# YannDubs/lossyless

Hardware: AMD Instinct MI355X
Metric: encode_img_per_sec (higher is better)
Workload: dtype f16; 1 GPU; clip_compressor_b005 encode, synthetic 224x224x3 fp16 NHWC, batch=1024/GPU (configs[1]); batch_per_gpu=1024, layout=nhwc, vit_weights=synthetic-seed1, parallelism=image-parallel x1, entropy_group=16, tower_batch=8704, tower_streams=1, distinct_batches=9

## Files before the change

lossyless_amd/csrc/gemm_w8_kernel.h:

```cpp
#pragma once
#include "gemm_common.h"

namespace lla {
namespace {

constexpr int kWStage = 65536, kWARegion = 32768;
constexpr int kWBiasOff = 2 * kWStage, kWBiasBytes = 3072 * 4;
#ifndef LLA_W8_GROUP_M
#define LLA_W8_GROUP_M 4
#endif
#ifndef LLA_W8_DMA_N0
#define LLA_W8_DMA_N0 5
#endif
#ifndef LLA_W8_DMA_N1
#define LLA_W8_DMA_N1 13
#endif

struct WItem { int kind, idx, d; };
constexpr WItem w_item(int p, int k) {
  return p == 0 ? WItem{0, 2 + k, 1} : p == 1 ? WItem{1, k, 2} : p == 2 ? WItem{1, 2 + k, 2} : WItem{0, k, 2};
}
constexpr int w_confirm(int p) {
  int seq = 0, last_a[14][4] = {}, last_b[14] = {}, upto[14][4] = {};
  for (int t = -2; t < 10; ++t)
    for (int q = 0; q < 4; ++q) {
      for (int k = 0; k < 2; ++k) {
        const WItem it = w_item(q, k);
        const int u = t + it.d;
        ++seq;
        if (u >= 0 && u < 14) { if (it.kind == 0) last_a[u][it.idx] = seq; else last_b[u] = seq; }
      }
      if (t >= 0) upto[t][q] = seq;
    }
  const int t = 4;
  int need = 0;
  if (p == 0) need = last_a[t][2];
  if (p == 1) need = last_a[t][3];
  if (p == 2) need = last_a[t + 1][0] > last_b[t + 1] ? last_a[t + 1][0] : last_b[t + 1];
  if (p == 3) need = last_a[t + 1][1];
  return upto[t][p] - need;
}
static_assert(w_confirm(0) == 9 && w_confirm(1) == 10 && w_confirm(2) == 7 && w_confirm(3) == 8, "schedule / wait counts out of step");
constexpr int w_confirm_pipe(int kind, int p, int n0, int n1) {
  const int TL = 6;
  int seq = 0, last_a[16][4] = {}, last_b[16] = {}, upto[16][4] = {};
  for (int t = 0; t < 12; ++t)
    for (int q = 0; q < 4; ++q) {
      const bool stores = (t == TL && q >= 1) || (t == TL + 1 && q == 0);
      for (int n = 0; n < 16; ++n) {
        if (n == n0 || n == n1) {
          const WItem it = w_item(q, n == n1 ? 1 : 0);
          const int u = t + it.d;
          ++seq;
          if (it.kind == 0) last_a[u][it.idx] = seq; else last_b[u] = seq;
        }
        if (stores && (n & 3) == 3) ++seq;
      }
      upto[t][q] = seq;
    }
  const int t = kind == 1 ? TL : kind == 2 ? TL + 1 : 3;
  int need = 0;
  if (p == 0) need = last_a[t][2];
  if (p == 1) need = last_a[t][3];
  if (p == 2) need = last_a[t + 1][0] > last_b[t + 1] ? last_a[t + 1][0] : last_b[t + 1];
  if (p == 3) need = last_a[t + 1][1];
  return upto[t][p] - need;
}
static_assert(w_confirm_pipe(0, 0, 5, 13) == 9 && w_confirm_pipe(0, 1, 5, 13) == 10 && w_confirm_pipe(0, 2, 5, 13) == 7 &&
              w_confirm_pipe(0, 3, 5, 13) == 8, "the replayed stream and the schedule table must agree where there are no stores");
static_assert(w_confirm_pipe(1, 0, 5, 13) == 9 && w_confirm_pipe(1, 1, 5, 13) == 14 && w_confirm_pipe(1, 2, 5, 13) == 15 &&
              w_confirm_pipe(1, 3, 5, 13) == 20 && w_confirm_pipe(2, 0, 5, 13) == 25 && w_confirm_pipe(2, 1, 5, 13) == 26 &&
              w_confirm_pipe(2, 2, 5, 13) == 14 && w_confirm_pipe(2, 3, 5, 13) == 13, "hand count of the default placement");

template <int... I, class F>
__device__ __forceinline__ void w_static_for_impl(std::integer_sequence<int, I...>, F &&f) { (f(std::integral_constant<int, I>{}), ...); }
template <int N, class F>
__device__ __forceinline__ void w_static_for(F &&f) { w_static_for_impl(std::make_integer_sequence<int, N>{}, f); }

typedef unsigned w_rsrc_t __attribute__((ext_vector_type(4)));
template <int IMM>
__device__ __forceinline__ void w_dma(unsigned voff, w_rsrc_t rsrc, unsigned soff, unsigned lds_base) {
  asm volatile("s_add_u32 m0, %3, %4\n\t"
               "s_nop 0\n\t"
               "buffer_load_dwordx4 %0, %1, %2 offen" LLA_DMA_SC " lds"
               :
               : "v"(voff), "s"(rsrc), "s"(soff), "s"(lds_base), "n"(IMM)
               : "memory", "m0", "scc");
}
__device__ __forceinline__ void w_dma_flat(unsigned voff, const unsigned char *sbase, unsigned lds_dst) {
  asm volatile("s_mov_b32 m0, %2\n\t"
               "s_nop 0\n\t"
               "global_load_lds_dwordx4 %0, %1"
               :
               : "v"(voff), "s"(sbase), "s"(lds_dst)
               : "memory", "m0");
}

#define LLA_W8_WAIT_VM(C) __builtin_amdgcn_s_waitcnt(0x0F70 | ((C) & 15) | (((C) >> 4) << 14))

template <int EPI, int DBG = 0, int PIPE = 0>
__global__ __launch_bounds__(512) void gemm_w8_kernel(GemmParams p) {
  static_assert(EPI == EPI_F16 || EPI == EPI_QGELU, "fp16 outputs only");
  constexpr bool kPipe = PIPE != 0 && DBG == 0;
  kernel_acquire();
  __shared__ __attribute__((aligned(16))) unsigned char smem[kWBiasOff + kWBiasBytes];

  const int tid = threadIdx.x, lane = tid & 63;
  const int wid = __builtin_amdgcn_readfirstlane(tid >> 6);
  const int wr = wid >> 2, wc = wid & 3;
  const int r16 = lane & 15, kq = lane >> 4;

  const int tiles_n = p.N / 256, tiles_m = (p.M + 255) / 256;
  const int total = tiles_m * tiles_n;
  const int bid = blockIdx.x, nblk = gridDim.x;
  const int xcd = bid & 7, slot = bid >> 3;
  const int nslots = (nblk - xcd + 7) >> 3;
  const int tq = total >> 3, tr = total & 7;
  const int start = xcd < tr ? xcd * (tq + 1) : tr * (tq + 1) + (xcd - tr) * tq;
  const int count = tq + (xcd < tr ? 1 : 0);
  const int n_my = slot < count ? (count - slot + nslots - 1) / nslots : 0;
  if (n_my == 0) return;
  constexpr int group_m = LLA_W8_GROUP_M;
  auto tile_origin = [&](int j, int &m0, int &n0) {
    int logical = start + slot + j * nslots;
    if (p.rev) logical = total - 1 - logical;
    const int per_group = group_m * tiles_n;
    const int grp = logical / per_group;
    const int in_grp = logical - grp * per_group;
    const int gh = (tiles_m - grp * group_m) < group_m ? (tiles_m - grp * group_m) : group_m;
    const int tn = in_grp / gh;
    m0 = (grp * group_m + (in_grp - tn * gh)) * 256;
    n0 = tn * 256;
  };
  const int nk = p.K / 64;

  const int pc = lane & 7, lc = pc ^ (((wid & 1) << 2) | (lane >> 4));
  const int rowA = (wid >> 2) * 128 + (wid & 3) * 8 + (lane >> 3);
  const int rowB = wid * 8 + (lane >> 3);
  unsigned voffA[4], voffB[4];
#pragma unroll
  for (int a = 0; a < 4; ++a) {
    voffA[a] = (unsigned)((rowA + 32 * a) * p.lda + lc * 8) * 2u;
    voffB[a] = (unsigned)((rowB + 64 * a) * p.K + lc * 8) * 2u;
  }
  const unsigned lds_base = (unsigned)(uintptr_t)(lptr_t)smem;
  const unsigned dstA = __builtin_amdgcn_readfirstlane(lds_base + (unsigned)((wid >> 2) * 16384 + (wid & 3) * 1024));
  const unsigned dstB = __builtin_amdgcn_readfirstlane(lds_base + (unsigned)(kWARegion + wid * 1024));
  auto make_rsrc = [](const void *base) {
    const unsigned long long a = reinterpret_cast<unsigned long long>(base);
    w_rsrc_t r = {(unsigned)__builtin_amdgcn_readfirstlane((unsigned)a),
                  (unsigned)__builtin_amdgcn_readfirstlane((unsigned)(a >> 32)) & 0xFFFFu, 0xFFFFFFFFu, 0x00020000u};
    return r;
  };
  const w_rsrc_t rsrcA = make_rsrc(p.A), rsrcB = make_rsrc(p.W);
  unsigned srcA[2], srcB[2];
  int cur_j = 0, cur_kt = 0;
  auto src_of = [&](int j, int kt, unsigned &a, unsigned &b) {
    int m0, n0;
    tile_origin(j < n_my ? j : n_my - 1, m0, n0);
    if (m0 + 256 > p.M) m0 = p.M >= 256 ? p.M - 256 : 0;
    a = __builtin_amdgcn_readfirstlane((unsigned)(((size_t)m0 * p.lda + (size_t)kt * 64) * 2));
    b = __builtin_amdgcn_readfirstlane((unsigned)(((size_t)n0 * p.K + (size_t)kt * 64) * 2));
  };
  auto advance_cursor = [&] {
    if (DBG == 15) return;
    srcA[0] = srcA[1]; srcB[0] = srcB[1];
    if (++cur_kt < nk) { srcA[1] += 128; srcB[1] += 128; }
    else { cur_kt = 0; ++cur_j; src_of(cur_j, 0, srcA[1], srcB[1]); }
  };
  if (p.M < 256) {
#pragma unroll
    for (int a = 0; a < 4; ++a) {
      const int r = rowA + 32 * a;
      voffA[a] = (unsigned)((r < p.M ? r : p.M - 1) * p.lda + lc * 8) * 2u;
    }
  }
  auto issue = [&](auto kind_c, auto idx_c, int d, unsigned st_off) {
    constexpr int kind = decltype(kind_c)::value, idx = decltype(idx_c)::value;
    if constexpr (kind == 0) w_dma<idx * 4096>(voffA[idx], rsrcA, srcA[d - 1], dstA + st_off);
    else w_dma<idx * 8192>(voffB[idx], rsrcB, srcB[d - 1], dstB + st_off);
  };
  using I0 = std::integral_constant<int, 0>; using I1 = std::integral_constant<int, 1>;
  using I2 = std::integral_constant<int, 2>; using I3 = std::integral_constant<int, 3>;

  unsigned a_off[2], b_off[2];
#pragma unroll
  for (int s = 0; s < 2; ++s) {
    const unsigned c = (unsigned)(((4 * s + kq) ^ ((r16 >> 1) & 7)) * 16);
    a_off[s] = (unsigned)((wr * 128 + r16) * 128) + c;
    b_off[s] = (unsigned)kWARegion + (unsigned)((wc * 64 + r16) * 128) + c;
  }
  f16x8 gb[4][2], ga[2][2];
  f32x4 acc[8][4];
  auto read_a = [&](unsigned so, int frag, int af, int s) {
    ga[af][s] = *reinterpret_cast<const f16x8 *>(smem + so + a_off[s] + frag * 2048);
  };
  auto read_b = [&](unsigned so, int b, int s) {
    gb[b][s] = *reinterpret_cast<const f16x8 *>(smem + so + b_off[s] + b * 2048);
  };

  if (p.bias) {
    for (int q = wid; q * 256 < p.N; q += 8)
      w_dma_flat((unsigned)lane * 16u, reinterpret_cast<const unsigned char *>(p.bias) + (size_t)q * 1024,
                 __builtin_amdgcn_readfirstlane(lds_base + (unsigned)kWBiasOff + (unsigned)q * 1024u));
  } else {
    for (int i = tid; i * 16 < p.N * 4; i += 512) *reinterpret_cast<f32x4 *>(smem + kWBiasOff + i * 16) = f32x4{0.f, 0.f, 0.f, 0.f};
  }
  src_of(0, 0, srcA[1], srcB[1]);
  srcA[0] = srcA[1]; srcB[0] = srcB[1];
  issue(I0{}, I0{}, 2, 0u); issue(I0{}, I1{}, 2, 0u); issue(I0{}, I2{}, 2, 0u); issue(I0{}, I3{}, 2, 0u);
  issue(I1{}, I0{}, 2, 0u); issue(I1{}, I1{}, 2, 0u); issue(I1{}, I2{}, 2, 0u); issue(I1{}, I3{}, 2, 0u);
  advance_cursor();
  issue(I1{}, I0{}, 2, (unsigned)kWStage); issue(I1{}, I1{}, 2, (unsigned)kWStage);
  issue(I1{}, I2{}, 2, (unsigned)kWStage); issue(I1{}, I3{}, 2, (unsigned)kWStage);
  issue(I0{}, I0{}, 2, (unsigned)kWStage); issue(I0{}, I1{}, 2, (unsigned)kWStage);
  advance_cursor();
  LLA_W8_WAIT_VM(6);
  asm volatile("" ::: "memory");
  __builtin_amdgcn_s_barrier();
  asm volatile("" ::: "memory");
#pragma unroll
  for (int b = 0; b < 4; ++b) read_b(0u, b, 0);
  read_a(0u, 0, 0, 0); read_a(0u, 1, 1, 0); read_a(0u, 0, 0, 1);

  int it = 0;

  typedef unsigned u32x4 __attribute__((ext_vector_type(4)));
  f32x4 ebias[4];
  unsigned char *ecrow = nullptr;
  unsigned elive = 0;
  unsigned ebias_off = 0;
  const size_t e_f_step = (size_t)16 * p.ldc * 2;
  auto epi_setup = [&](int cj) {
    int m0c, n0c;
    tile_origin(cj, m0c, n0c);
    unsigned ones = ~0u;
    asm volatile("" : "+s"(ones));
    const int el = (int)__builtin_amdgcn_mbcnt_hi(ones, __builtin_amdgcn_mbcnt_lo(ones, 0u));
    const int er = el & 15, eq = el >> 4;
    int mbase = m0c, mskip = 0;
    if (m0c + 256 > p.M) { mbase = p.M >= 256 ? p.M - 256 : 0; mskip = m0c - mbase; }
    const int nw = n0c + wc * 64;
    const int rl0 = wr * 128 + er;
    const int col = 16 * (eq & 1) + 8 * (eq >> 1);
    elive = 0;
#pragma unroll
    for (int f = 0; f < 8; ++f) elive |= (rl0 + 16 * f >= mskip && mbase + rl0 + 16 * f < p.M) ? (1u << f) : 0u;
    ecrow = reinterpret_cast<unsigned char *>(reinterpret_cast<f16 *>(p.C) + (size_t)(mbase + rl0) * p.ldc + nw + col);
    ebias_off = (unsigned)(nw + 4 * eq) * 4u;
  };
  auto epi_bias = [&](int b) {
    ebias[b] = *reinterpret_cast<const f32x4 *>(smem + kWBiasOff + ebias_off + 64 * b);
  };
  auto epi_frag = [&](int f) {
    u32x4 o[2];
#pragma unroll
    for (int bp = 0; bp < 4; bp += 2) {
      unsigned lo[2], hi[2];
#pragma unroll
      for (int h = 0; h < 2; ++h) {
        f32x4 v = acc[f][bp + h];
        asm volatile("" : "+v"(v));
        v += ebias[bp + h];
        if constexpr (EPI == EPI_QGELU) {
#pragma unroll
          for (int e = 0; e < 4; ++e) v[e] = quick_gelu(v[e]);
        }
        typedef f16 f16x2 __attribute__((ext_vector_type(2)));
        const f16x2 a2 = {(f16)v[0], (f16)v[1]}, b2 = {(f16)v[2], (f16)v[3]};
        lo[h] = __builtin_bit_cast(unsigned, a2);
        hi[h] = __builtin_bit_cast(unsigned, b2);
      }
      const auto rx = __builtin_amdgcn_permlane16_swap(lo[0], lo[1], false, false);
      const auto ry = __builtin_amdgcn_permlane16_swap(hi[0], hi[1], false, false);
      o[bp >> 1] = u32x4{rx[0], ry[0], rx[1], ry[1]};
    }
    if constexpr (DBG == 5) asm volatile("" ::"v"(o[0]), "v"(o[1]));
    else if ((elive >> f) & 1u) { store16(ecrow + f * e_f_step, o[0]); store16(ecrow + f * e_f_step + 64, o[1]); }
  };

  auto ktile = [&](auto first_c, auto last_c, auto pend_c) {
    constexpr bool FIRST = decltype(first_c)::value, LAST = decltype(last_c)::value, PEND = decltype(pend_c)::value;
    unsigned so = (unsigned)(it & 1) * kWStage, sn = (unsigned)((it + 1) & 1) * kWStage;
    w_static_for<4>([&](auto a_c) {
      constexpr int a = decltype(a_c)::value;
      __builtin_amdgcn_sched_barrier(0);
      if (DBG != 2) __builtin_amdgcn_s_barrier();
      __builtin_amdgcn_sched_barrier(0);
      asm volatile("" : "+s"(so), "+s"(sn));
      w_static_for<16>([&](auto n_c) {
        constexpr int n = decltype(n_c)::value;
        constexpr int g = n >> 2, b = n & 3, s = g >> 1, af = g & 1;
        if constexpr (FIRST && s == 0) {
          const f32x4 zero4 = {0.f, 0.f, 0.f, 0.f};
          acc[2 * a + af][b] = __builtin_amdgcn_mfma_f32_16x16x32_f16(gb[b][0], ga[af][0], zero4, 0, 0, 0);
        } else {
          acc[2 * a + af][b] = __builtin_amdgcn_mfma_f32_16x16x32_f16(gb[b][s], ga[af][s], acc[2 * a + af][b], 0, 0, 0);
        }
        __builtin_amdgcn_sched_barrier(0);
        if constexpr (b == 0) {
          constexpr int pg = (g + 3) & 3, ps = pg >> 1, paf = pg & 1;
          if constexpr (g == 0) read_a(so, 2 * a + paf, paf, ps);
          else if constexpr (a < 3) read_a(so, 2 * (a + 1) + paf, paf, ps);
          else read_a(sn, paf, paf, ps);
        }
        if constexpr (a == 0 && n < 4) read_b(so, n, 1);
        if constexpr (a == 3 && n >= 8 && n < 12) read_b(sn, n - 8, 0);
        if constexpr (DBG != 1 && DBG != 13 && (n == LLA_W8_DMA_N0 || n == LLA_W8_DMA_N1)) {
          constexpr WItem item = w_item(a, n == LLA_W8_DMA_N1 ? 1 : 0);
          issue(std::integral_constant<int, item.kind>{}, std::integral_constant<int, item.idx>{}, item.d,
                (unsigned)((it + item.d) & 1) * kWStage);
        }
        if constexpr (kPipe && (LAST || PEND)) {
          if constexpr (LAST && a == 0) { if constexpr ((n & 3) == 3) epi_bias(n >> 2); }
          else if constexpr ((n & 7) == 7) {
            if constexpr (LAST) epi_frag(2 * (a - 1) + (n >> 3));
            else if constexpr (a == 0) epi_frag(6 + (n >> 3));
          }
        }
        __builtin_amdgcn_sched_barrier(0);
      });
      if (DBG != 4) {
        constexpr int kind = !kPipe ? 0 : LAST ? 1 : PEND ? 2 : 0;
        constexpr int cf = w_confirm_pipe(kind, a, LLA_W8_DMA_N0, LLA_W8_DMA_N1);
        static_assert(cf <= 63, "vmcnt is a 6-bit field");
        LLA_W8_WAIT_VM(cf);
      }
      asm volatile("" ::: "memory");
    });
    ++it;
    advance_cursor();
  };
  using T_ = std::integral_constant<bool, true>;
  using F_ = std::integral_constant<bool, false>;

  for (int cj = 0; cj < n_my; ++cj) {
    if constexpr (kPipe) {
      if (cj == 0) ktile(T_{}, F_{}, F_{});
      else ktile(T_{}, F_{}, T_{});
      for (int kt = 1; kt < nk - 1; ++kt) ktile(F_{}, F_{}, F_{});
      epi_setup(cj);
      ktile(F_{}, T_{}, F_{});
      continue;
    }
    ktile(T_{}, F_{}, F_{});
    for (int kt = 1; kt < nk; ++kt) ktile(F_{}, F_{}, F_{});
    asm volatile("" ::: "memory");
    if constexpr (DBG == 3 || DBG == 13 || DBG == 15) {
      unsigned ones = ~0u;
      asm volatile("" : "+s"(ones));
      const int el = (int)__builtin_amdgcn_mbcnt_hi(ones, __builtin_amdgcn_mbcnt_lo(ones, 0u));
      float t = 0.f;
#pragma unroll
      for (int f = 0; f < 8; ++f)
#pragma unroll
        for (int b = 0; b < 4; ++b) t += acc[f][b][0] + acc[f][b][1] + acc[f][b][2] + acc[f][b][3];
      if (t == 1.2345e30f) reinterpret_cast<f16 *>(p.C)[el] = (f16)t;
    } else {
      epi_setup(cj);
#pragma unroll
      for (int b = 0; b < 4; ++b) epi_bias(b);
#pragma unroll
      for (int f = 0; f < 8; ++f) epi_frag(f);
    }
    asm volatile("" ::: "memory");
  }
  if constexpr (kPipe) {
    epi_frag(6); epi_frag(7);
  }
  __builtin_amdgcn_s_waitcnt(0x0070);
  kernel_release();
}


}
}
```

Baseline: 107,700 img/s.

## Halve workgroup barriers per K-tile in W8 GEMM by re-planning DMA schedule

Cuts the s_barrier and vmcnt waits in the 8-wave GEMM main loop from four per K-tile to two (at phases 1 and 3). The LDS DMA item schedule is reassigned so every write-after-read and read-after-write hazard is still covered by the remaining barriers, and a constexpr replay checks legality and computes the wait counts. The aim is to reduce barrier stalls between waves. In exchange, loads must land earlier and some waits get tighter, and the old four-barrier schedule stays available behind a macro.

```diff
diff --git a/lossyless_amd/csrc/gemm_w8_kernel.h b/lossyless_amd/csrc/gemm_w8_kernel.h
--- a/lossyless_amd/csrc/gemm_w8_kernel.h
+++ b/lossyless_amd/csrc/gemm_w8_kernel.h
@@ -16,61 +16,89 @@
 #define LLA_W8_DMA_N1 13
 #endif
 
+#ifndef LLA_W8_SYNC4
+#define LLA_W8_SYNC4 0
+#endif
+constexpr bool w_meets(int p) { return LLA_W8_SYNC4 ? true : (p & 1) != 0; }
+
 struct WItem { int kind, idx, d; };
+#if LLA_W8_SYNC4
+constexpr int w_nitems(int) { return 2; }
 constexpr WItem w_item(int p, int k) {
   return p == 0 ? WItem{0, 2 + k, 1} : p == 1 ? WItem{1, k, 2} : p == 2 ? WItem{1, 2 + k, 2} : WItem{0, k, 2};
 }
-constexpr int w_confirm(int p) {
-  int seq = 0, last_a[14][4] = {}, last_b[14] = {}, upto[14][4] = {};
-  for (int t = -2; t < 10; ++t)
-    for (int q = 0; q < 4; ++q) {
-      for (int k = 0; k < 2; ++k) {
-        const WItem it = w_item(q, k);
-        const int u = t + it.d;
-        ++seq;
-        if (u >= 0 && u < 14) { if (it.kind == 0) last_a[u][it.idx] = seq; else last_b[u] = seq; }
-      }
-      if (t >= 0) upto[t][q] = seq;
-    }
-  const int t = 4;
-  int need = 0;
-  if (p == 0) need = last_a[t][2];
-  if (p == 1) need = last_a[t][3];
-  if (p == 2) need = last_a[t + 1][0] > last_b[t + 1] ? last_a[t + 1][0] : last_b[t + 1];
-  if (p == 3) need = last_a[t + 1][1];
-  return upto[t][p] - need;
-}
-static_assert(w_confirm(0) == 9 && w_confirm(1) == 10 && w_confirm(2) == 7 && w_confirm(3) == 8, "schedule / wait counts out of step");
-constexpr int w_confirm_pipe(int kind, int p, int n0, int n1) {
+#else
+constexpr int w_nitems(int p) { return p == 0 ? 1 : p == 1 ? 3 : 2; }
+constexpr WItem w_item(int p, int k) {
+  return p == 0 ? WItem{0, 2, 1} : p == 1 ? (k == 0 ? WItem{0, 3, 1} : WItem{1, k - 1, 2}) : p == 2 ? WItem{1, 2 + k, 2} : WItem{0, 1 - k, 2};
+}
+#endif
+constexpr int w_pos(int p, int k, int n0, int n1) {
+  return w_nitems(p) == 1 ? (n0 + n1) / 2 : w_nitems(p) == 2 ? (k == 0 ? n0 : n1) : (k == 0 ? n0 : k == 1 ? (n0 + n1) / 2 : n1);
+}
+constexpr int w_prologue() {
+  int n = 0;
+  for (int p = 0; p < 4; ++p)
+    for (int k = 0; k < w_nitems(p); ++k) n += w_item(p, k).d == 2 ? 1 : 0;
+  return n;
+}
+
+struct WReplay { int cf[4]; bool legal; };
+constexpr WReplay w_replay(int kind, int n0, int n1) {
   const int TL = 6;
-  int seq = 0, last_a[16][4] = {}, last_b[16] = {}, upto[16][4] = {};
+  int seq = 0, stamp[16][8] = {}, upto[64] = {};
+  bool legal = true;
   for (int t = 0; t < 12; ++t)
     for (int q = 0; q < 4; ++q) {
       const bool stores = (t == TL && q >= 1) || (t == TL + 1 && q == 0);
       for (int n = 0; n < 16; ++n) {
-        if (n == n0 || n == n1) {
-          const WItem it = w_item(q, n == n1 ? 1 : 0);
-          const int u = t + it.d;
-          ++seq;
-          if (it.kind == 0) last_a[u][it.idx] = seq; else last_b[u] = seq;
-        }
+        for (int k = 0; k < w_nitems(q); ++k)
+          if (w_pos(q, k, n0, n1) == n) {
+            const WItem it = w_item(q, k);
+            const int u = t + it.d, piece = it.kind == 0 ? it.idx : 4 + it.idx;
+            stamp[u][piece] = ++seq;
+            const int last_read = 4 * (u - 2) + (it.kind == 0 ? it.idx : 0);
+            bool met = false;
+            for (int g = last_read + 1; g <= 4 * t + q; ++g) met = met || w_meets(g & 3);
+            legal = legal && met;
+          }
         if (stores && (n & 3) == 3) ++seq;
       }
-      upto[t][q] = seq;
+      upto[4 * t + q] = seq;
     }
   const int t = kind == 1 ? TL : kind == 2 ? TL + 1 : 3;
-  int need = 0;
-  if (p == 0) need = last_a[t][2];
-  if (p == 1) need = last_a[t][3];
-  if (p == 2) need = last_a[t + 1][0] > last_b[t + 1] ? last_a[t + 1][0] : last_b[t + 1];
-  if (p == 3) need = last_a[t + 1][1];
-  return upto[t][p] - need;
-}
-static_assert(w_confirm_pipe(0, 0, 5, 13) == 9 && w_confirm_pipe(0, 1, 5, 13) == 10 && w_confirm_pipe(0, 2, 5, 13) == 7 &&
-              w_confirm_pipe(0, 3, 5, 13) == 8, "the replayed stream and the schedule table must agree where there are no stores");
-static_assert(w_confirm_pipe(1, 0, 5, 13) == 9 && w_confirm_pipe(1, 1, 5, 13) == 14 && w_confirm_pipe(1, 2, 5, 13) == 15 &&
-              w_confirm_pipe(1, 3, 5, 13) == 20 && w_confirm_pipe(2, 0, 5, 13) == 25 && w_confirm_pipe(2, 1, 5, 13) == 26 &&
-              w_confirm_pipe(2, 2, 5, 13) == 14 && w_confirm_pipe(2, 3, 5, 13) == 13, "hand count of the default placement");
+  WReplay r{{-1, -1, -1, -1}, legal};
+  for (int p = 0; p < 4; ++p) {
+    if (!w_meets((p + 1) & 3)) continue;
+    int need = 0;
+    for (int g = 4 * t + p + 1; g == 4 * t + p + 1 || !w_meets(g & 3); ++g)
+      for (int u = t; u <= t + 2; ++u)
+        for (int piece = 0; piece < 8; ++piece) {
+          const int first_read = 4 * u + (piece < 4 ? piece - 1 : -1);
+          if (first_read != g) continue;
+          if (stamp[u][piece] == 0 || stamp[u][piece] > upto[4 * t + p]) r.legal = false;
+          if (stamp[u][piece] > need) need = stamp[u][piece];
+        }
+    r.cf[p] = upto[4 * t + p] - need;
+    if (need == 0 || r.cf[p] < 0 || r.cf[p] > 63) r.legal = false;
+  }
+  int once[8] = {};
+  for (int q = 0; q < 4; ++q)
+    for (int k = 0; k < w_nitems(q); ++k) ++once[w_item(q, k).kind == 0 ? w_item(q, k).idx : 4 + w_item(q, k).idx];
+  for (int piece = 0; piece < 8; ++piece) r.legal = r.legal && once[piece] == 1;
+  return r;
+}
+constexpr bool w_replay_ok(int n0, int n1) { return w_replay(0, n0, n1).legal && w_replay(1, n0, n1).legal && w_replay(2, n0, n1).legal; }
+static_assert(w_replay_ok(5, 13) && w_replay_ok(2, 10) && w_replay_ok(7, 15), "DMA schedule: a WAR or RAW rule is broken");
+#if LLA_W8_SYNC4
+static_assert(w_replay(0, 5, 13).cf[0] == 9 && w_replay(0, 5, 13).cf[1] == 10 && w_replay(0, 5, 13).cf[2] == 7 &&
+              w_replay(0, 5, 13).cf[3] == 8, "schedule / wait counts out of step");
+static_assert(w_replay(1, 5, 13).cf[0] == 9 && w_replay(1, 5, 13).cf[1] == 14 && w_replay(1, 5, 13).cf[2] == 15 &&
+              w_replay(1, 5, 13).cf[3] == 20 && w_replay(2, 5, 13).cf[0] == 25 && w_replay(2, 5, 13).cf[1] == 26 &&
+              w_replay(2, 5, 13).cf[2] == 14 && w_replay(2, 5, 13).cf[3] == 13, "hand count of the default placement");
+#else
+static_assert(w_replay(0, 5, 13).cf[1] < 0 && w_replay(0, 5, 13).cf[3] < 0, "two periods per K-tile: waits close phases 0 and 2 only");
+#endif
 
 template <int... I, class F>
 __device__ __forceinline__ void w_static_for_impl(std::integer_sequence<int, I...>, F &&f) { (f(std::integral_constant<int, I>{}), ...); }
@@ -211,11 +239,16 @@
   issue(I0{}, I0{}, 2, 0u); issue(I0{}, I1{}, 2, 0u); issue(I0{}, I2{}, 2, 0u); issue(I0{}, I3{}, 2, 0u);
   issue(I1{}, I0{}, 2, 0u); issue(I1{}, I1{}, 2, 0u); issue(I1{}, I2{}, 2, 0u); issue(I1{}, I3{}, 2, 0u);
   advance_cursor();
-  issue(I1{}, I0{}, 2, (unsigned)kWStage); issue(I1{}, I1{}, 2, (unsigned)kWStage);
-  issue(I1{}, I2{}, 2, (unsigned)kWStage); issue(I1{}, I3{}, 2, (unsigned)kWStage);
-  issue(I0{}, I0{}, 2, (unsigned)kWStage); issue(I0{}, I1{}, 2, (unsigned)kWStage);
+  w_static_for<4>([&](auto q_c) {
+    constexpr int q = decltype(q_c)::value;
+    w_static_for<w_nitems(q)>([&](auto k_c) {
+      constexpr WItem item = w_item(q, decltype(k_c)::value);
+      if constexpr (item.d == 2)
+        issue(std::integral_constant<int, item.kind>{}, std::integral_constant<int, item.idx>{}, 2, (unsigned)kWStage);
+    });
+  });
   advance_cursor();
-  LLA_W8_WAIT_VM(6);
+  LLA_W8_WAIT_VM(w_prologue());
   asm volatile("" ::: "memory");
   __builtin_amdgcn_s_barrier();
   asm volatile("" ::: "memory");
@@ -285,7 +318,7 @@
     w_static_for<4>([&](auto a_c) {
       constexpr int a = decltype(a_c)::value;
       __builtin_amdgcn_sched_barrier(0);
-      if (DBG != 2) __builtin_amdgcn_s_barrier();
+      if constexpr (DBG != 2 && w_meets(a)) __builtin_amdgcn_s_barrier();
       __builtin_amdgcn_sched_barrier(0);
       asm volatile("" : "+s"(so), "+s"(sn));
       w_static_for<16>([&](auto n_c) {
@@ -306,10 +339,15 @@
         }
         if constexpr (a == 0 && n < 4) read_b(so, n, 1);
         if constexpr (a == 3 && n >= 8 && n < 12) read_b(sn, n - 8, 0);
-        if constexpr (DBG != 1 && DBG != 13 && (n == LLA_W8_DMA_N0 || n == LLA_W8_DMA_N1)) {
-          constexpr WItem item = w_item(a, n == LLA_W8_DMA_N1 ? 1 : 0);
-          issue(std::integral_constant<int, item.kind>{}, std::integral_constant<int, item.idx>{}, item.d,
-                (unsigned)((it + item.d) & 1) * kWStage);
+        if constexpr (DBG != 1 && DBG != 13) {
+          w_static_for<w_nitems(a)>([&](auto k_c) {
+            constexpr int k = decltype(k_c)::value;
+            if constexpr (w_pos(a, k, LLA_W8_DMA_N0, LLA_W8_DMA_N1) == n) {
+              constexpr WItem item = w_item(a, k);
+              issue(std::integral_constant<int, item.kind>{}, std::integral_constant<int, item.idx>{}, item.d,
+                    (unsigned)((it + item.d) & 1) * kWStage);
+            }
+          });
         }
         if constexpr (kPipe && (LAST || PEND)) {
           if constexpr (LAST && a == 0) { if constexpr ((n & 3) == 3) epi_bias(n >> 2); }
@@ -320,11 +358,11 @@
         }
         __builtin_amdgcn_sched_barrier(0);
       });
-      if (DBG != 4) {
+      if constexpr (DBG != 4 && w_meets((a + 1) & 3)) {
         constexpr int kind = !kPipe ? 0 : LAST ? 1 : PEND ? 2 : 0;
-        constexpr int cf = w_confirm_pipe(kind, a, LLA_W8_DMA_N0, LLA_W8_DMA_N1);
-        static_assert(cf <= 63, "vmcnt is a 6-bit field");
-        LLA_W8_WAIT_VM(cf);
+        constexpr WReplay rp = w_replay(kind, LLA_W8_DMA_N0, LLA_W8_DMA_N1);
+        static_assert(rp.legal && rp.cf[a] >= 0 && rp.cf[a] <= 63, "vmcnt is a 6-bit field");
+        LLA_W8_WAIT_VM(rp.cf[a]);
       }
       asm volatile("" ::: "memory");
     });
```

New measurement: 108,400 img/s (median of 6 runs). No clear change (+0.6%).
